# lyclyc52/Instance_NeRF

Measured on AMD Instinct MI355X. Metric: Msamples/sec (train+infer) 3D-FRONT 800x800 at 1/2/4/8 MI355X; PSNR parity, higher is better.
Workload: dtype f32; 1 GPU; render 800x800 synthetic 3D-FRONT-like room, hash-grid NeRF L=16 F=2 T=6119864 sigma+rgb (BASELINE configs[1]), one view per step per GPU; parallelism=views sharded over 1 GPU(s), no data-path collective

## Files before the change

instance_nerf_amd/build.py:

```python
import os
import shutil
import subprocess
import sys

HERE = os.path.dirname(os.path.abspath(__file__))
CSRC = os.path.join(HERE, "csrc")
LIB = os.path.join(CSRC, "libinr_hip.so")
SOURCES = ["raymarch.hip", "encoders.hip", "field_fused.hip", "roialign.hip", "mesh.hip", "components.hip", "match.hip",
           "overlap.hip"]
HEADERS = ["common.h", "grid_common.h", os.path.join("..", "..", "include", "inr.h")]
FLAGS = ["--offload-arch=gfx950", "-O3", "-std=c++17", "-fPIC", "-ffp-contract=off",
         "-munsafe-fp-atomics", "-Wall", "-Wno-unused-function"]


KERNEL_FILES = {
    "field": ["field_fused.hip", "common.h", "grid_common.h"],
    "scatter": ["encoders.hip", "common.h", "grid_common.h"],
}


def source_sha(kind=None):
    import hashlib
    h = hashlib.sha256()
    for f in sorted(KERNEL_FILES[kind] if kind else SOURCES + HEADERS):
        h.update(f.encode())
        h.update(open(os.path.join(CSRC, f), "rb").read())
    return h.hexdigest()


LIB_FP32 = os.path.join(CSRC, "libinr_hip_fp32.so")


def build_fp32(force=False, verbose=True):
    deps = [os.path.join(CSRC, f) for f in SOURCES + HEADERS] + [os.path.abspath(__file__)]
    if not force and os.path.exists(LIB_FP32) and all(os.path.getmtime(d) <= os.path.getmtime(LIB_FP32) for d in deps):
        return LIB_FP32
    hipcc = shutil.which("hipcc") or "/opt/rocm/bin/hipcc"
    objs = []
    for src in SOURCES:
        obj = os.path.join(CSRC, src.replace(".hip", ".fp32.o"))
        cmd = [hipcc, "-x", "hip", "-c", os.path.join(CSRC, src), "-o", obj, "-DINR_MLP_FP32=1"] + FLAGS
        if verbose:
            print(" ".join(cmd), flush=True)
        subprocess.check_call(cmd)
        objs.append(obj)
    subprocess.check_call([hipcc, "-shared", "-o", LIB_FP32] + objs + ["--offload-arch=gfx950"])
    return LIB_FP32


def _stale():
    if not os.path.exists(LIB):
        return True
    t = os.path.getmtime(LIB)
    deps = [os.path.join(CSRC, f) for f in SOURCES + HEADERS] + [os.path.abspath(__file__)]
    return any(os.path.getmtime(d) > t for d in deps)


def build(force=False, verbose=True):
    if not force and not _stale():
        return LIB
    hipcc = shutil.which("hipcc") or "/opt/rocm/bin/hipcc"
    if not os.path.exists(hipcc):
        raise RuntimeError("hipcc not found: cannot build libinr_hip.so")
    objs = []
    for src in SOURCES:
        obj = os.path.join(CSRC, src.replace(".hip", ".o"))
        cmd = [hipcc, "-x", "hip", "-c", os.path.join(CSRC, src), "-o", obj] + FLAGS
        if verbose:
            print(" ".join(cmd), flush=True)
        subprocess.check_call(cmd)
        objs.append(obj)
    cmd = [hipcc, "-shared", "-o", LIB] + objs + ["--offload-arch=gfx950"]
    if verbose:
        print(" ".join(cmd), flush=True)
    subprocess.check_call(cmd)
    return LIB


if __name__ == "__main__":
    build(force="--force" in sys.argv)
    build_fp32(force="--force" in sys.argv)
    print(LIB)
```

instance_nerf_amd/csrc/raymarch.hip:

```cpp
#include "common.h"

namespace inr {

static thread_local char g_err[512] = "";
int g_field_lds_min = 0;
int g_march_lds_pad = 0;
void set_error(const char* fmt, ...) {
  va_list ap;
  va_start(ap, fmt);
  vsnprintf(g_err, sizeof(g_err), fmt, ap);
  va_end(ap);
}

constexpr int kRayBlock = 256;
constexpr float kSqrt3x2 = 3.4641016151377544f;

__global__ void __launch_bounds__(kRayBlock) k_near_far(const float* __restrict__ rays_o,
                                                        const float* __restrict__ rays_d,
                                                        const float* __restrict__ aabb, int64_t N,
                                                        float min_near, float* __restrict__ nears,
                                                        float* __restrict__ fars,
                                                        const int64_t* __restrict__ labels, int64_t ignore) {
  const int64_t n = (int64_t)blockIdx.x * blockDim.x + threadIdx.x;
  if (n >= N) return;
  float near = -INFINITY, far = INFINITY;
  bool miss = labels != nullptr && labels[n] == ignore;
#pragma unroll
  for (int a = 0; a < 3; ++a) {
    const float o = rays_o[n * 3 + a];
    const float rd = 1.0f / rays_d[n * 3 + a];
    const float t0 = (aabb[a] - o) * rd;
    const float t1 = (aabb[a + 3] - o) * rd;
    const float lo = t0 > t1 ? t1 : t0;
    const float hi = t0 > t1 ? t0 : t1;
    if (a > 0) miss = miss || (near > hi) || (lo > far);
    near = lo > near ? lo : near;
    far = hi < far ? hi : far;
  }
  if (near < min_near) near = min_near;
  nears[n] = miss ? 3.402823466e+38f : near;
  fars[n] = miss ? 3.402823466e+38f : far;
}

__global__ void __launch_bounds__(kRayBlock) k_get_rays(const float* __restrict__ poses, int64_t B, float fx, float fy,
                                                        float cx, float cy, int W, const int64_t* __restrict__ inds,
                                                        int64_t n, float* __restrict__ rays_o,
                                                        float* __restrict__ rays_d) {
  const int64_t idx = (int64_t)blockIdx.x * blockDim.x + threadIdx.x;
  if (idx >= B * n) return;
  const int64_t b = idx / n, k = idx - b * n;
  const int64_t pix = inds ? inds[k] : k;
  const float i = (float)(pix % W) + 0.5f, j = (float)(pix / W) + 0.5f;
  const float xs = (i - cx) / fx, ys = (j - cy) / fy;
  const float nrm = sqrtf(xs * xs + ys * ys + 1.0f * 1.0f);
  const float dx = xs / nrm, dy = ys / nrm, dz = 1.0f / nrm;
  const float* P = poses + b * 16;
#pragma unroll
  for (int r = 0; r < 3; ++r) {
    rays_d[idx * 3 + r] = dx * P[r * 4 + 0] + dy * P[r * 4 + 1] + dz * P[r * 4 + 2];
    rays_o[idx * 3 + r] = P[r * 4 + 3];
  }
}

__device__ __forceinline__ uint64_t mix64(uint64_t z) {
  z = (z ^ (z >> 30)) * 0xBF58476D1CE4E5B9ull;
  z = (z ^ (z >> 27)) * 0x94D049BB133111EBull;
  return z ^ (z >> 31);
}
__global__ void __launch_bounds__(kRayBlock) k_sample_batch(const float* __restrict__ pose, float fx, float fy, float cx,
                                                            float cy, int H, int W, const float* __restrict__ image,
                                                            int C, const int32_t* __restrict__ mask, int num_instances,
                                                            uint64_t seed, uint64_t step, int64_t n,
                                                            int64_t* __restrict__ inds, float* __restrict__ rays_o,
                                                            float* __restrict__ rays_d, float* __restrict__ rgb,
                                                            int64_t* __restrict__ labels) {
  const int64_t k = (int64_t)blockIdx.x * blockDim.x + threadIdx.x;
  if (k >= n) return;
  const uint64_t h = mix64(seed + 0x9E3779B97F4A7C15ull * ((step << 32) + (uint64_t)k));
  const uint64_t pix = ((h >> 32) * (uint64_t)((int64_t)H * W)) >> 32;
  inds[k] = (int64_t)pix;
  const float i = (float)(pix % (uint64_t)W) + 0.5f, j = (float)(pix / (uint64_t)W) + 0.5f;
  const float xs = (i - cx) / fx, ys = (j - cy) / fy;
  const float nrm = sqrtf(xs * xs + ys * ys + 1.0f * 1.0f);
  const float dx = xs / nrm, dy = ys / nrm, dz = 1.0f / nrm;
#pragma unroll
  for (int r = 0; r < 3; ++r) {
    rays_d[k * 3 + r] = dx * pose[r * 4 + 0] + dy * pose[r * 4 + 1] + dz * pose[r * 4 + 2];
    rays_o[k * 3 + r] = pose[r * 4 + 3];
  }
  if (image) {
    for (int c = 0; c < C; ++c) rgb[k * C + c] = image[pix * C + c];
  }
  if (mask) {
    const int32_t l = mask[pix];
    labels[k] = l >= num_instances ? -1 : (int64_t)l;
  }
}

__global__ void k_morton3D(const int32_t* __restrict__ coords, int64_t N, int32_t* __restrict__ out) {
  const int64_t n = (int64_t)blockIdx.x * blockDim.x + threadIdx.x;
  if (n >= N) return;
  out[n] = (int32_t)morton3((uint32_t)coords[n * 3], (uint32_t)coords[n * 3 + 1], (uint32_t)coords[n * 3 + 2]);
}
__global__ void k_morton3D_invert(const int32_t* __restrict__ idx, int64_t N, int32_t* __restrict__ coords) {
  const int64_t n = (int64_t)blockIdx.x * blockDim.x + threadIdx.x;
  if (n >= N) return;
  const uint32_t m = (uint32_t)idx[n];
  coords[n * 3 + 0] = (int32_t)compact_bits10(m);
  coords[n * 3 + 1] = (int32_t)compact_bits10(m >> 1);
  coords[n * 3 + 2] = (int32_t)compact_bits10(m >> 2);
}
__global__ void k_packbits(const float* __restrict__ grid, int64_t n_bytes, float thresh,
                           uint8_t* __restrict__ bits) {
  const int64_t n = (int64_t)blockIdx.x * blockDim.x + threadIdx.x;
  if (n >= n_bytes) return;
  const float4 a = reinterpret_cast<const float4*>(grid)[n * 2];
  const float4 b = reinterpret_cast<const float4*>(grid)[n * 2 + 1];
  uint32_t v = (a.x > thresh) | ((a.y > thresh) << 1) | ((a.z > thresh) << 2) | ((a.w > thresh) << 3) |
               ((b.x > thresh) << 4) | ((b.y > thresh) << 5) | ((b.z > thresh) << 6) | ((b.w > thresh) << 7);
  bits[n] = (uint8_t)v;
}

__global__ void k_occ_positions(const int32_t* __restrict__ morton, const float* __restrict__ noise, int64_t n, float Hm1,
                                float ext, float half, float* __restrict__ xyz) {
  const int64_t i = (int64_t)blockIdx.x * blockDim.x + threadIdx.x;
  if (i >= n) return;
  const uint32_t m = morton ? (uint32_t)morton[i] : (uint32_t)i;
  const uint32_t c[3] = {compact_bits10(m), compact_bits10(m >> 1), compact_bits10(m >> 2)};
#pragma unroll
  for (int a = 0; a < 3; ++a) {
    float v = (2.0f * (float)c[a] / Hm1 - 1.0f) * ext;
    if (noise) v = v + (noise[i * 3 + a] * 2.0f - 1.0f) * half;
    xyz[i * 3 + a] = v;
  }
}
__global__ void __launch_bounds__(256) k_mark_untrained(const float* __restrict__ poses, int B, float kx, float ky, int H,
                                                        int C, float bound, float* __restrict__ grid) {
  const int64_t i = (int64_t)blockIdx.x * blockDim.x + threadIdx.x;
  const int64_t H3 = (int64_t)H * H * H;
  if (i >= (int64_t)C * H3) return;
  const int cas = (int)(i / H3);
  const uint32_t m = (uint32_t)(i - (int64_t)cas * H3);
  const float bnd = fminf(ldexpf(1.0f, cas), bound), half = bnd / (float)H, ext = bnd - half;
  const float wx = (2.0f * (float)compact_bits10(m) / (float)(H - 1) - 1.0f) * ext;
  const float wy = (2.0f * (float)compact_bits10(m >> 1) / (float)(H - 1) - 1.0f) * ext;
  const float wz = (2.0f * (float)compact_bits10(m >> 2) / (float)(H - 1) - 1.0f) * ext;
  bool seen = false;
  for (int b = 0; b < B && !seen; ++b) {
    const float* P = poses + (int64_t)b * 16;
    const float dx = wx - P[3], dy = wy - P[7], dz = wz - P[11];
    const float cx = dx * P[0] + dy * P[4] + dz * P[8];
    const float cy = dx * P[1] + dy * P[5] + dz * P[9];
    const float cz = dx * P[2] + dy * P[6] + dz * P[10];
    seen = cz > 0.0f && fabsf(cx) < kx * cz + half * 2.0f && fabsf(cy) < ky * cz + half * 2.0f;
  }
  if (!seen) grid[i] = -1.0f;
}

__global__ void k_occ_scatter(const float* __restrict__ sigma, const int32_t* __restrict__ morton, int64_t m,
                              float density_scale, float* __restrict__ tmp) {
  const int64_t i = (int64_t)blockIdx.x * blockDim.x + threadIdx.x;
  if (i < m) tmp[morton[i]] = sigma[i] * density_scale;
}
__global__ void __launch_bounds__(256) k_occ_update(float* __restrict__ grid, const float* __restrict__ tmp, int64_t n,
                                                    float decay, float scale, double* __restrict__ mean_sum) {
  __shared__ double red[4];
  double acc = 0.0;
  auto cell = [&](float g, float t, bool& changed) {
    t *= scale;
    if (g >= 0.0f && t >= 0.0f) { g = fmaxf(g * decay, t); changed = true; }
    acc += (double)fmaxf(g, 0.0f);
    return g;
  };
  const int64_t n4 = (((uintptr_t)grid | (uintptr_t)tmp) & 15) == 0 ? n / 4 : 0;
  for (int64_t i = (int64_t)blockIdx.x * blockDim.x + threadIdx.x; i < n4; i += (int64_t)gridDim.x * blockDim.x) {
    float4 g = reinterpret_cast<float4*>(grid)[i];
    const float4 t = reinterpret_cast<const float4*>(tmp)[i];
    bool changed = false;
    g.x = cell(g.x, t.x, changed); g.y = cell(g.y, t.y, changed); g.z = cell(g.z, t.z, changed); g.w = cell(g.w, t.w, changed);
    if (changed) reinterpret_cast<float4*>(grid)[i] = g;
  }
  for (int64_t i = n4 * 4 + (int64_t)blockIdx.x * blockDim.x + threadIdx.x; i < n; i += (int64_t)gridDim.x * blockDim.x) {
    bool changed = false;
    const float g = cell(grid[i], tmp[i], changed);
    if (changed) grid[i] = g;
  }
#pragma unroll
  for (int d = 32; d >= 1; d >>= 1) acc += __shfl_xor(acc, d, 64);
  if ((threadIdx.x & 63) == 0) red[threadIdx.x >> 6] = acc;
  __syncthreads();
  if (threadIdx.x == 0) atomicAdd(mean_sum, red[0] + red[1] + red[2] + red[3]);
}
__global__ void k_packbits_mean(const float* __restrict__ grid, int64_t n_bytes, const double* __restrict__ mean_sum,
                                double inv_cells, float density_thresh, uint8_t* __restrict__ bits,
                                float* __restrict__ mean_out, const int32_t* __restrict__ counters, int n_counters,
                                int counter_stride, double* __restrict__ stats_out) {
  const int64_t n = (int64_t)blockIdx.x * blockDim.x + threadIdx.x;
  const float mean = (float)(*mean_sum * inv_cells);
  if (n == 0 && mean_out) *mean_out = mean;
  if (n == 0 && stats_out) {
    int64_t total = 0;
    for (int k = 0; k < n_counters; ++k) total += counters[(int64_t)k * counter_stride];
    stats_out[0] = (double)mean;
    stats_out[1] = (double)total;
  }
  if (n >= n_bytes) return;
  const float thresh = fminf(mean, density_thresh);
  const float4 a = reinterpret_cast<const float4*>(grid)[n * 2];
  const float4 b = reinterpret_cast<const float4*>(grid)[n * 2 + 1];
  uint32_t v = (a.x > thresh) | ((a.y > thresh) << 1) | ((a.z > thresh) << 2) | ((a.w > thresh) << 3) |
               ((b.x > thresh) << 4) | ((b.y > thresh) << 5) | ((b.z > thresh) << 6) | ((b.w > thresh) << 7);
  bits[n] = (uint8_t)v;
}

struct MarchParams {
  const uint8_t* bits;
  float bound, dt_gamma, dt_min, dt_max, rH;
  int C, H, H3;
};

struct Ray {
  float ox, oy, oz, dx, dy, dz, rdx, rdy, rdz, sx, sy, sz;
};

__device__ __forceinline__ Ray load_ray(const float* __restrict__ o, const float* __restrict__ d, int64_t n) {
  Ray r;
  r.ox = o[n * 3]; r.oy = o[n * 3 + 1]; r.oz = o[n * 3 + 2];
  r.dx = d[n * 3]; r.dy = d[n * 3 + 1]; r.dz = d[n * 3 + 2];
  r.rdx = 1.0f / r.dx; r.rdy = 1.0f / r.dy; r.rdz = 1.0f / r.dz;
  r.sx = copysignf(1.0f, r.dx); r.sy = copysignf(1.0f, r.dy); r.sz = copysignf(1.0f, r.dz);
  return r;
}

__device__ __forceinline__ float step_dt(const MarchParams& P, float t) {
  return clampf(t * P.dt_gamma, P.dt_min, P.dt_max);
}
template <bool kConst>
struct StepRule {
  float c;
  __device__ __forceinline__ explicit StepRule(const MarchParams& P) : c(step_dt(P, 0.0f)) {}
  __device__ __forceinline__ float operator()(const MarchParams& P, float t) const {
    if constexpr (kConst) return c;
    else return step_dt(P, t);
  }
};

struct MortonCalc {
  __device__ __forceinline__ uint32_t operator()(uint32_t x, uint32_t y, uint32_t z) const { return morton3(x, y, z); }
};
struct MortonLut {
  const uint32_t* lut;
  __device__ __forceinline__ uint32_t operator()(uint32_t x, uint32_t y, uint32_t z) const {
    return lut[x] | (lut[y] << 1) | (lut[z] << 2);
  }
};

template <bool kSingle = false, bool kConstDt = false, class Emit, class Advance, class Morton = MortonCalc>
__device__ __forceinline__ int march_ray(const MarchParams& P, const Ray& r, float t, float far,
                                         int max_emit, Emit&& emit, Advance&& advance, Morton morton = Morton()) {
  int n = 0;
  float last_t = t;
  const StepRule<kConstDt> step(P);
  const float mb1 = fminf(ldexpf(1.0f, 0), P.bound), rmb1 = 1.0f / mb1;
  while (t < far && n < max_emit) {
    const float px = clampf(r.ox + t * r.dx, -P.bound, P.bound);
    const float py = clampf(r.oy + t * r.dy, -P.bound, P.bound);
    const float pz = clampf(r.oz + t * r.dz, -P.bound, P.bound);
    const float dt = step(P, t);
    int level = 0;
    float mb = mb1, rmb = rmb1;
    if constexpr (!kSingle) {
      int e0, e1;
      (void)frexpf(fmaxf(fabsf(px), fmaxf(fabsf(py), fabsf(pz))), &e0);
      (void)frexpf(dt * (float)P.H * 0.5f, &e1);
      level = max(clampi(e0, 0, P.C - 1), clampi(e1, 0, P.C - 1));
      mb = fminf(ldexpf(1.0f, level), P.bound);
      rmb = 1.0f / mb;
    }
    const int nx = clampi((int)(((px * rmb + 1.0f) * 0.5f) * (float)P.H), 0, P.H - 1);
    const int ny = clampi((int)(((py * rmb + 1.0f) * 0.5f) * (float)P.H), 0, P.H - 1);
    const int nz = clampi((int)(((pz * rmb + 1.0f) * 0.5f) * (float)P.H), 0, P.H - 1);
    const uint32_t idx = (uint32_t)level * (uint32_t)P.H3 + morton((uint32_t)nx, (uint32_t)ny, (uint32_t)nz);
    const bool occ = (P.bits[idx >> 3] >> (idx & 7)) & 1;
    if (occ) {
      const float tn = t + dt;
      emit(px, py, pz, dt, tn - last_t, t);
      t = tn;
      advance();
      last_t = tn;
      ++n;
    } else {
      const float ax = ((float)nx + 0.5f) + 0.5f * r.sx;
      const float ay = ((float)ny + 0.5f) + 0.5f * r.sy;
      const float az = ((float)nz + 0.5f) + 0.5f * r.sz;
      const float cx = (((ax * P.rH) * 2.0f - 1.0f) * mb - px) * r.rdx;
      const float cy = (((ay * P.rH) * 2.0f - 1.0f) * mb - py) * r.rdy;
      const float cz = (((az * P.rH) * 2.0f - 1.0f) * mb - pz) * r.rdz;
      const float tt = t + fmaxf(0.0f, fminf(cx, fminf(cy, cz)));
      do {
        t = t + step(P, t);
        advance();
      } while (t < tt);
    }
  }
  return n;
}
template <class Emit>
__device__ __forceinline__ int march_ray(const MarchParams& P, const Ray& r, float t, float far,
                                         int max_emit, Emit&& emit) {
  return P.dt_gamma == 0.0f ? march_ray<false, true>(P, r, t, far, max_emit, emit, [] {})
                            : march_ray<false, false>(P, r, t, far, max_emit, emit, [] {});
}
template <class Emit, class Advance, class Morton>
__device__ __forceinline__ int march_ray_any(const MarchParams& P, const Ray& r, float t, float far,
                                             int max_emit, Emit&& emit, Advance&& advance, Morton morton) {
  if (P.dt_gamma == 0.0f)
    return P.C == 1 ? march_ray<true, true>(P, r, t, far, max_emit, emit, advance, morton)
                    : march_ray<false, true>(P, r, t, far, max_emit, emit, advance, morton);
  return P.C == 1 ? march_ray<true, false>(P, r, t, far, max_emit, emit, advance, morton)
                  : march_ray<false, false>(P, r, t, far, max_emit, emit, advance, morton);
}

__device__ __forceinline__ float start_t(const MarchParams& P, float near, float noise) {
  return near + step_dt(P, near) * noise;
}

__global__ void __launch_bounds__(kRayBlock) k_march_count(MarchParams P, const float* __restrict__ rays_o,
                                                           const float* __restrict__ rays_d, int64_t N,
                                                           int max_steps, const float* __restrict__ nears,
                                                           const float* __restrict__ fars,
                                                           const float* __restrict__ noises,
                                                           int32_t* __restrict__ counts,
                                                           int32_t* __restrict__ block_sums,
                                                           uint32_t* __restrict__ mask, int cap_words) {
  __shared__ int32_t wsum[kRayBlock / 64];
  __shared__ uint32_t lut[1024];
  for (int i = threadIdx.x; i < P.H; i += kRayBlock) lut[i] = expand_bits10((uint32_t)i);
  __syncthreads();
  const MortonLut morton{lut};
  const int64_t n = (int64_t)blockIdx.x * blockDim.x + threadIdx.x;
  int cnt = 0;
  if (n < N) {
    const Ray r = load_ray(rays_o, rays_d, n);
    const float t0 = start_t(P, nears[n], noises ? noises[n] : 0.0f);
    if (cap_words > 0) {
      uint32_t word = 0;
      int widx = 0, cand = 0;
      bool ok = true;
      cnt = march_ray_any(P, r, t0, fars[n], max_steps,
                      [&](float, float, float, float, float, float) {
                        const int w = cand >> 5;
                        if (w < cap_words) {
                          while (widx < w) {
                            mask[(int64_t)widx * N + n] = word;
                            word = 0;
                            ++widx;
                          }
                          word |= 1u << (cand & 31);
                        } else {
                          ok = false;
                        }
                      },
                      [&] { ++cand; }, morton);
      if (widx < cap_words) mask[(int64_t)widx * N + n] = word;
      mask[(int64_t)cap_words * N + n] = ok ? 1u : 0u;
    } else {
      cnt = march_ray_any(P, r, t0, fars[n], max_steps, [](float, float, float, float, float, float) {}, [] {}, morton);
    }
    counts[n] = cnt;
  }
  const int incl = wave_inclusive_scan(cnt);
  if ((threadIdx.x & 63) == 63) wsum[threadIdx.x >> 6] = incl;
  __syncthreads();
  if (threadIdx.x == 0) {
    int s = 0;
#pragma unroll
    for (int w = 0; w < kRayBlock / 64; ++w) s += wsum[w];
    block_sums[blockIdx.x] = s;
  }
}

__global__ void __launch_bounds__(1024) k_scan_block_sums(int32_t* __restrict__ block_sums, int n_blocks,
                                                          int64_t N, int32_t* __restrict__ counter) {
  __shared__ int32_t wsum[16];
  __shared__ int32_t carry_s;
  if (threadIdx.x == 0) carry_s = 0;
  __syncthreads();
  for (int base = 0; base < n_blocks; base += 1024) {
    const int i = base + threadIdx.x;
    const int v = i < n_blocks ? block_sums[i] : 0;
    const int incl = wave_inclusive_scan(v);
    if ((threadIdx.x & 63) == 63) wsum[threadIdx.x >> 6] = incl;
    __syncthreads();
    int wave_off = 0;
    for (int w = 0; w < (int)(threadIdx.x >> 6); ++w) wave_off += wsum[w];
    const int carry = carry_s;
    if (i < n_blocks) block_sums[i] = carry + wave_off + incl - v;
    __syncthreads();
    if (threadIdx.x == 1023) carry_s = carry + wave_off + incl;
    __syncthreads();
  }
  if (threadIdx.x == 0) {
    counter[0] = carry_s;
    counter[1] = (int32_t)N;
  }
}

__global__ void __launch_bounds__(kRayBlock) k_finalize_offsets(const int32_t* __restrict__ counts,
                                                                const int32_t* __restrict__ block_prefix,
                                                                int64_t N, int32_t* __restrict__ rays) {
  __shared__ int32_t wsum[kRayBlock / 64];
  const int64_t n = (int64_t)blockIdx.x * blockDim.x + threadIdx.x;
  const int cnt = n < N ? counts[n] : 0;
  const int incl = wave_inclusive_scan(cnt);
  if ((threadIdx.x & 63) == 63) wsum[threadIdx.x >> 6] = incl;
  __syncthreads();
  int off = block_prefix[blockIdx.x] + incl - cnt;
  for (int w = 0; w < (int)(threadIdx.x >> 6); ++w) off += wsum[w];
  if (n < N) {
    rays[n * 3 + 0] = (int32_t)n;
    rays[n * 3 + 1] = off;
    rays[n * 3 + 2] = cnt;
  }
}

template <bool kConstDt, class Emit>
__device__ __forceinline__ void replay_ray_t(const MarchParams& P, const Ray& r, const uint32_t* __restrict__ mask, int64_t N,
                                             int64_t n, float t, int cnt, Emit&& emit) {
  const StepRule<kConstDt> step(P);
  float last_t = t;
  int emitted = 0;
  for (int w = 0; emitted < cnt; ++w) {
    const uint32_t bits = mask[(int64_t)w * N + n];
    for (int b0 = 0; b0 < 32; b0 += 8) {
      const uint32_t sub = (bits >> b0) & 0xFFu;
      if (__ballot(sub != 0u) == 0ull) {
#pragma unroll
        for (int j = 0; j < 8; ++j) t = t + step(P, t);
        continue;
      }
#pragma unroll
      for (int j = 0; j < 8; ++j) {
        const float dt = step(P, t);
        const float tn = t + dt;
        if (sub & (1u << j)) {
          const float px = clampf(r.ox + t * r.dx, -P.bound, P.bound);
          const float py = clampf(r.oy + t * r.dy, -P.bound, P.bound);
          const float pz = clampf(r.oz + t * r.dz, -P.bound, P.bound);
          emit(px, py, pz, dt, tn - last_t, t);
          last_t = tn;
          ++emitted;
        }
        t = tn;
      }
    }
  }
}
template <class Emit>
__device__ __forceinline__ void replay_ray(const MarchParams& P, const Ray& r, const uint32_t* __restrict__ mask, int64_t N,
                                           int64_t n, float t, int cnt, Emit&& emit) {
  if (P.dt_gamma == 0.0f) replay_ray_t<true>(P, r, mask, N, n, t, cnt, emit);
  else replay_ray_t<false>(P, r, mask, N, n, t, cnt, emit);
}

__global__ void __launch_bounds__(kRayBlock) k_march_write(MarchParams P, const float* __restrict__ rays_o,
                                                           const float* __restrict__ rays_d, int64_t N,
                                                           int64_t M, const float* __restrict__ nears,
                                                           const float* __restrict__ fars,
                                                           const float* __restrict__ noises,
                                                           const int32_t* __restrict__ rays,
                                                           float* __restrict__ xyzs, float* __restrict__ dirs,
                                                           float* __restrict__ deltas,
                                                           const uint32_t* __restrict__ mask, int cap_words) {
  const int64_t n = (int64_t)blockIdx.x * blockDim.x + threadIdx.x;
  if (n >= N) return;
  const int off = rays[n * 3 + 1];
  const int cnt = rays[n * 3 + 2];
  if (cnt == 0 || (int64_t)off + cnt > M) return;
  const Ray r = load_ray(rays_o, rays_d, n);
  int64_t i = off;
  auto emit = [&](float px, float py, float pz, float dt, float delta, float) {
    xyzs[i * 3 + 0] = px; xyzs[i * 3 + 1] = py; xyzs[i * 3 + 2] = pz;
    dirs[i * 3 + 0] = r.dx; dirs[i * 3 + 1] = r.dy; dirs[i * 3 + 2] = r.dz;
    deltas[i * 2 + 0] = dt; deltas[i * 2 + 1] = delta;
    ++i;
  };
  const float t0 = start_t(P, nears[n], noises ? noises[n] : 0.0f);
  if (cap_words > 0 && mask[(int64_t)cap_words * N + n]) {
    replay_ray(P, r, mask, N, n, t0, cnt, emit);
  } else {
    march_ray(P, r, t0, fars[n], cnt, emit);
  }
}

template <bool kSingle = false, class Emit>
__device__ __forceinline__ int march_ray_coop(const MarchParams& P, const Ray& r, float t, float far, int max_emit,
                                              Emit&& emit) {
  const float mb1 = fminf(ldexpf(1.0f, 0), P.bound), rmb1 = 1.0f / mb1;
  const int lane = threadIdx.x & 63;
  const uint64_t lt_mask = (1ull << lane) - 1ull;
  int n = 0;
  float last_t = t;
  while (t < far && n < max_emit) {
    float c = t;
    if (P.dt_gamma == 0.0f) {
      const float dt0 = step_dt(P, t);
      asm volatile(
          ".rept 63\n"
          "s_nop 1\n"
          "v_add_f32_dpp %0, %0, %1 wave_shr:1 row_mask:0xf bank_mask:0xf\n"
          ".endr\n"
          : "+v"(c)
          : "v"(dt0));
    } else {
      for (int j = 0; j < 63; ++j) c = j < lane ? c + step_dt(P, c) : c;
    }
    const bool in = c < far;
    const float px = clampf(r.ox + c * r.dx, -P.bound, P.bound);
    const float py = clampf(r.oy + c * r.dy, -P.bound, P.bound);
    const float pz = clampf(r.oz + c * r.dz, -P.bound, P.bound);
    const float dt = step_dt(P, c);
    const float tn = c + dt;
    int level = 0;
    float mb = mb1, rmb = rmb1;
    if constexpr (!kSingle) {
      int e0, e1;
      (void)frexpf(fmaxf(fabsf(px), fmaxf(fabsf(py), fabsf(pz))), &e0);
      (void)frexpf(dt * (float)P.H * 0.5f, &e1);
      level = max(clampi(e0, 0, P.C - 1), clampi(e1, 0, P.C - 1));
      mb = fminf(ldexpf(1.0f, level), P.bound);
      rmb = 1.0f / mb;
    }
    const int nx = clampi((int)(((px * rmb + 1.0f) * 0.5f) * (float)P.H), 0, P.H - 1);
    const int ny = clampi((int)(((py * rmb + 1.0f) * 0.5f) * (float)P.H), 0, P.H - 1);
    const int nz = clampi((int)(((pz * rmb + 1.0f) * 0.5f) * (float)P.H), 0, P.H - 1);
    const uint32_t idx = (uint32_t)level * (uint32_t)P.H3 + morton3((uint32_t)nx, (uint32_t)ny, (uint32_t)nz);
    const bool occ = (P.bits[idx >> 3] >> (idx & 7)) & 1;
    const float ax = ((float)nx + 0.5f) + 0.5f * r.sx;
    const float ay = ((float)ny + 0.5f) + 0.5f * r.sy;
    const float az = ((float)nz + 0.5f) + 0.5f * r.sz;
    const float cx = (((ax * P.rH) * 2.0f - 1.0f) * mb - px) * r.rdx;
    const float cy = (((ay * P.rH) * 2.0f - 1.0f) * mb - py) * r.rdy;
    const float cz = (((az * P.rH) * 2.0f - 1.0f) * mb - pz) * r.rdz;
    const float tt = c + fmaxf(0.0f, fminf(cx, fminf(cy, cz)));
    int lo = lane + 1, hi = 64;
    bool settled_all = false;
    if (P.dt_gamma == 0.0f) {
      const int i0 = lane + (int)fminf((tt - c) * (1.0f / dt), 64.0f);
      const float ca = __shfl(c, clampi(i0 - 1, 0, 63), 64);
      const float cb = __shfl(c, min(i0, 63), 64);
      const float cc = __shfl(c, min(i0 + 1, 63), 64);
      const bool lt_a = i0 - 1 <= lane || ca < tt;
      const bool ge_b = i0 >= 64 || !(cb < tt);
      const bool ge_c = i0 + 1 >= 64 || !(cc < tt);
      const bool take_b = i0 > lane && ge_b;
      const bool settled = take_b ? lt_a : ge_c;
      lo = take_b ? min(i0, 64) : i0 + 1;
      settled_all = __ballot(in && !occ && !settled) == 0;
    }
    if (!settled_all) {
      lo = lane + 1;
#pragma unroll
      for (int it = 0; it < 7; ++it) {
        const int mid = (lo + hi) >> 1;
        const float cm = __shfl(c, min(mid, 63), 64);
        const bool below = mid < 64 && cm < tt;
        if (lo < hi) {
          if (below) lo = mid + 1; else hi = mid;
        }
      }
    }
    const int next = lo;
    const uint64_t in_mask = __ballot(in);
    const uint64_t miss_mask = __ballot(in && !occ);
    const int n_in = __popcll(in_mask);
    uint64_t visited = 0;
    int v = 0, last_miss = -1;
    while (v < n_in) {
      const uint64_t rest = miss_mask >> v;
      const int m = rest ? v + __builtin_ctzll(rest) : 64;
      const int stop = min(m, n_in);
      if (stop > v) visited |= (stop - v >= 64 ? ~0ull : ((1ull << (stop - v)) - 1ull)) << v;
      if (m >= n_in) { v = stop; last_miss = -1; break; }
      visited |= 1ull << m;
      last_miss = m;
      v = __builtin_amdgcn_readlane(next, m);
    }
    uint64_t emit_mask = visited & in_mask & ~miss_mask;
    int k_new = __popcll(emit_mask);
    bool full = false;
    if (n + k_new >= max_emit) {
      full = true;
      const int keep = max_emit - n;
      uint64_t m2 = emit_mask;
      for (int i = 0; i < keep; ++i) m2 &= m2 - 1;
      emit_mask &= ~m2;
      k_new = keep;
    }
    const uint64_t before = emit_mask & lt_mask;
    const int prev = before ? 63 - __builtin_clzll(before) : 0;
    const float prev_tn = __shfl(tn, prev, 64);
    if ((emit_mask >> lane) & 1ull) {
      const float last = before ? prev_tn : last_t;
      emit(n + __popcll(before), px, py, pz, dt, tn - last, c);
    }
    if (emit_mask) last_t = __builtin_bit_cast(float, __builtin_amdgcn_readlane(__builtin_bit_cast(int, tn),
                                                                                63 - __builtin_clzll(emit_mask)));
    n += k_new;
    if (full) break;
    if (v < 64) {
      t = far;
    } else {
      const float c63 = __builtin_bit_cast(float, __builtin_amdgcn_readlane(__builtin_bit_cast(int, tn), 63));
      t = c63;
      if (last_miss >= 0) {
        const float tt_m = __builtin_bit_cast(float, __builtin_amdgcn_readlane(__builtin_bit_cast(int, tt), last_miss));
        while (t < tt_m) t = t + step_dt(P, t);
      }
    }
  }
  return n;
}

constexpr int kCoopRaysPerBlock = 4;

__global__ void __launch_bounds__(kCoopRaysPerBlock * 64) k_march_count_coop(MarchParams P, const float* __restrict__ rays_o,
                                                                             const float* __restrict__ rays_d, int64_t N,
                                                                             int max_steps, const float* __restrict__ nears,
                                                                             const float* __restrict__ fars,
                                                                             const float* __restrict__ noises,
                                                                             int32_t* __restrict__ counts,
                                                                             float* __restrict__ stage, int stage_pitch) {
  const int64_t n = (int64_t)blockIdx.x * kCoopRaysPerBlock + (threadIdx.x >> 6);
  if (n >= N) return;
  const Ray r = load_ray(rays_o, rays_d, n);
  const float t0 = start_t(P, nears[n], noises ? noises[n] : 0.0f);
  int cnt;
  if (stage) {
    float* row = stage + (size_t)n * stage_pitch * 5;
    auto park = [&](int k, float px, float py, float pz, float dt, float delta, float) {
      float* q = row + (size_t)k * 5;
      q[0] = px; q[1] = py; q[2] = pz; q[3] = dt; q[4] = delta;
    };
    cnt = P.C == 1 ? march_ray_coop<true>(P, r, t0, fars[n], max_steps, park)
                   : march_ray_coop<false>(P, r, t0, fars[n], max_steps, park);
  } else {
    auto none = [](int, float, float, float, float, float, float) {};
    cnt = P.C == 1 ? march_ray_coop<true>(P, r, t0, fars[n], max_steps, none)
                   : march_ray_coop<false>(P, r, t0, fars[n], max_steps, none);
  }
  if ((threadIdx.x & 63) == 0) counts[n] = cnt;
}

__global__ void __launch_bounds__(kCoopRaysPerBlock * 64) k_march_write_staged(const float* __restrict__ rays_d, int64_t N,
                                                                               int64_t M, const int32_t* __restrict__ rays,
                                                                               const float* __restrict__ stage, int stage_pitch,
                                                                               float* __restrict__ xyzs, float* __restrict__ dirs,
                                                                               float* __restrict__ deltas) {
  const int64_t n = (int64_t)blockIdx.x * kCoopRaysPerBlock + (threadIdx.x >> 6);
  if (n >= N) return;
  const int off = rays[n * 3 + 1];
  const int cnt = rays[n * 3 + 2];
  const int lane = threadIdx.x & 63;
  auto zero_rows = [&](int64_t lo, int64_t hi) {
    for (int64_t i = lo + lane; i < hi; i += 64) {
      xyzs[i * 3 + 0] = 0.f; xyzs[i * 3 + 1] = 0.f; xyzs[i * 3 + 2] = 0.f;
      dirs[i * 3 + 0] = 0.f; dirs[i * 3 + 1] = 0.f; dirs[i * 3 + 2] = 0.f;
      deltas[i * 2 + 0] = 0.f; deltas[i * 2 + 1] = 0.f;
    }
  };
  const int64_t total = (int64_t)rays[(N - 1) * 3 + 1] + rays[(N - 1) * 3 + 2];
  if (total < M) {
    const int64_t per = (M - total + N - 1) / N;
    zero_rows(total + n * per, min(M, total + (n + 1) * per));
  }
  if ((int64_t)off + cnt > M) {
    if (cnt > 0 && off < M) zero_rows(off, M);
    return;
  }
  if (cnt == 0) return;
  const float dx = rays_d[n * 3], dy = rays_d[n * 3 + 1], dz = rays_d[n * 3 + 2];
  const float* row = stage + (size_t)n * stage_pitch * 5;
  for (int k = lane; k < cnt; k += 64) {
    const float* q = row + (size_t)k * 5;
    const int64_t i = (int64_t)off + k;
    xyzs[i * 3 + 0] = q[0]; xyzs[i * 3 + 1] = q[1]; xyzs[i * 3 + 2] = q[2];
    dirs[i * 3 + 0] = dx; dirs[i * 3 + 1] = dy; dirs[i * 3 + 2] = dz;
    deltas[i * 2 + 0] = q[3]; deltas[i * 2 + 1] = q[4];
  }
}

constexpr int kOccBuckets = 4096;
constexpr int kOccBlockCells = 1024;
constexpr int kOccMaxBlocks = 16384;
__global__ void __launch_bounds__(kOccBlockCells) k_occ_count(const float* __restrict__ grid, int64_t n_cells,
                                                              uint64_t* __restrict__ masks, int32_t* __restrict__ block_counts,
                                                              int32_t* __restrict__ hist) {
  __shared__ int32_t wcount[kOccBlockCells / 64];
  const int64_t i = (int64_t)blockIdx.x * kOccBlockCells + threadIdx.x;
  const uint64_t m = __ballot(i < n_cells && grid[i] > 0.0f);
  if ((threadIdx.x & 63) == 0) {
    masks[i >> 6] = m;
    wcount[threadIdx.x >> 6] = __popcll(m);
  }
  for (int64_t k = i; k < 2 * kOccBuckets; k += (int64_t)gridDim.x * kOccBlockCells) hist[k] = 0;
  __syncthreads();
  if (threadIdx.x == 0) {
    int c = 0;
    for (int w = 0; w < kOccBlockCells / 64; ++w) c += wcount[w];
    block_counts[blockIdx.x] = c;
  }
}
__global__ void __launch_bounds__(1024) k_occ_hist(const float* __restrict__ u, int64_t n, int32_t* __restrict__ hist) {
  __shared__ int32_t h[2 * kOccBuckets];
  for (int k = threadIdx.x; k < 2 * kOccBuckets; k += 1024) h[k] = 0;
  __syncthreads();
  for (int64_t j = (int64_t)blockIdx.x * 1024 + threadIdx.x; j < 2 * n; j += (int64_t)gridDim.x * 1024) {
    const int b = min((int)(u[j] * (float)kOccBuckets), kOccBuckets - 1);
    atomicAdd(&h[(j >= n ? kOccBuckets : 0) + b], 1);
  }
  __syncthreads();
  for (int k = threadIdx.x; k < 2 * kOccBuckets; k += 1024)
    if (h[k]) atomicAdd(&hist[k], h[k]);
}
__device__ void lds_exclusive_scan_1024(int32_t* a, int n, int32_t* wsum) {
  const int per = (n + 1023) / 1024;
  const int lo = min(n, (int)threadIdx.x * per), hi = min(n, lo + per);
  int s = 0;
  for (int i = lo; i < hi; ++i) s += a[i];
  const int incl = wave_inclusive_scan(s);
  if ((threadIdx.x & 63) == 63) wsum[threadIdx.x >> 6] = incl;
  __syncthreads();
// ... 1297 lines not shown
```

Baseline: 6442 Msamples/s.

## Replace per-step float marching in empty space with closed-form binade jumps

Adds a ConstStepper that, for constant step size, computes how many float additions of the step fit within the current exponent binade and jumps there in closed form using fma, so the result stays bit-exact with repeated t+=c. Empty-space skipping in march_ray and the mask replay in replay_ray_t use it, with replay jumping straight to each set bit via ctz instead of stepping through every candidate. The goal is to cut the long serial add loops over skipped samples. In exchange the per-ray code is more complex and branchy, and bit-exactness depends on subtle rounding handling.

```diff
diff --git a/instance_nerf_amd/build.py b/instance_nerf_amd/build.py
--- a/instance_nerf_amd/build.py
+++ b/instance_nerf_amd/build.py
@@ -8,7 +8,7 @@
 LIB = os.path.join(CSRC, "libinr_hip.so")
 SOURCES = ["raymarch.hip", "encoders.hip", "field_fused.hip", "roialign.hip", "mesh.hip", "components.hip", "match.hip",
            "overlap.hip"]
-HEADERS = ["common.h", "grid_common.h", os.path.join("..", "..", "include", "inr.h")]
+HEADERS = ["common.h", "grid_common.h", "const_step.h", os.path.join("..", "..", "include", "inr.h")]
 FLAGS = ["--offload-arch=gfx950", "-O3", "-std=c++17", "-fPIC", "-ffp-contract=off",
          "-munsafe-fp-atomics", "-Wall", "-Wno-unused-function"]
 
diff --git a/instance_nerf_amd/csrc/const_step.h b/instance_nerf_amd/csrc/const_step.h
--- /dev/null
+++ b/instance_nerf_amd/csrc/const_step.h
@@ -0,0 +1,126 @@
+#pragma once
+#include <math.h>
+#include <stdint.h>
+
+#if defined(__HIPCC__) || defined(__CUDACC__)
+#define INR_STEP_HD __host__ __device__ __forceinline__
+#else
+#define INR_STEP_HD inline
+#endif
+
+namespace inr {
+
+struct ConstStepper {
+  float c;
+  uint32_t eb = 0;
+  float q = 0.0f, rq = 0.0f, top = 0.0f;
+  bool plain = true;
+
+  static constexpr float kMaxJump = 32768.0f;
+
+  INR_STEP_HD explicit ConstStepper(float step) : c(step) {}
+
+  static INR_STEP_HD uint32_t bits_of(float x) {
+    uint32_t b;
+    __builtin_memcpy(&b, &x, sizeof b);
+    return b;
+  }
+  static INR_STEP_HD float float_of(uint32_t b) {
+    float x;
+    __builtin_memcpy(&x, &b, sizeof x);
+    return x;
+  }
+  static INR_STEP_HD bool covered(uint32_t e) { return e - 32u <= 190u; }
+
+  INR_STEP_HD void set_binade(uint32_t e) {
+    eb = e;
+    const float u = float_of((e - 23u) << 23), ru = float_of((277u - e) << 23);
+    top = float_of((e + 1u) << 23);
+    const float s = c * ru;
+    const float m = rintf(s);
+    q = m * u;
+    plain = !(fabsf(s - m) != 0.5f) || !(q > 0.0f);
+    rq = 1.0f / q;
+  }
+  INR_STEP_HD bool tie_or_stuck(uint32_t e) {
+    set_binade(e);
+    return plain;
+  }
+
+  INR_STEP_HD bool closed_form_at(float t, float* room) {
+    const uint32_t e = bits_of(t) >> 23;
+    if (!covered(e)) return false;
+    if (e != eb) set_binade(e);
+    *room = top - t;
+    return !plain && q <= *room;
+  }
+
+  INR_STEP_HD float advance_to(float t, float tt, int* steps) {
+    for (;;) {
+      float room;
+      if (!closed_form_at(t, &room)) {
+        t = t + c;
+        ++*steps;
+      } else {
+        const float lim = top < tt ? top : tt;
+        float kf = ceilf((lim - t) * rq);
+        kf = kf > 1.0f ? kf : 1.0f;
+        if (!(kf < kMaxJump)) {
+          t = t + c;
+          ++*steps;
+        } else {
+          float tk = fmaf(kf, q, t);
+          while (tk < lim) {
+            kf += 1.0f;
+            tk = fmaf(kf, q, t);
+          }
+          while (kf > 1.0f) {
+            const float tp = fmaf(kf - 1.0f, q, t);
+            if (!(tp >= lim)) break;
+            kf -= 1.0f;
+            tk = tp;
+          }
+          if (fmaf(kf, q, -room) > 0.0f) {
+            kf -= 1.0f;
+            t = fmaf(kf, q, t);
+            t = t + c;
+            *steps += (int)kf + 1;
+          } else {
+            t = tk;
+            *steps += (int)kf;
+          }
+        }
+      }
+      if (!(t < tt)) return t;
+    }
+  }
+
+  INR_STEP_HD float nth(float t, int k) {
+    while (k > 0) {
+      float room;
+      if (!closed_form_at(t, &room)) {
+        t = t + c;
+        --k;
+        continue;
+      }
+      const int kk = k < (int)kMaxJump ? k : (int)kMaxJump;
+      const float kf = (float)kk;
+      if (fmaf(kf, q, -room) <= 0.0f) {
+        t = fmaf(kf, q, t);
+        k -= kk;
+        continue;
+      }
+      float jf = floorf(room * rq);
+      jf = jf < kf - 1.0f ? jf : kf - 1.0f;
+      jf = jf > 1.0f ? jf : 1.0f;
+      while (fmaf(jf, q, -room) > 0.0f) jf -= 1.0f;
+      while (fmaf(jf + 1.0f, q, -room) <= 0.0f) jf += 1.0f;
+      t = fmaf(jf, q, t);
+      t = t + c;
+      k -= (int)jf + 1;
+    }
+    return t;
+  }
+};
+
+}
diff --git a/instance_nerf_amd/csrc/raymarch.hip b/instance_nerf_amd/csrc/raymarch.hip
--- a/instance_nerf_amd/csrc/raymarch.hip
+++ b/instance_nerf_amd/csrc/raymarch.hip
@@ -1,4 +1,7 @@
+#include <type_traits>
+
 #include "common.h"
+#include "const_step.h"
 
 namespace inr {
 
@@ -255,12 +258,19 @@
   }
 };
 
+template <class Advance>
+__device__ __forceinline__ void advance_by(Advance&& advance, int k) {
+  if constexpr (std::is_invocable_v<Advance&, int>) advance(k);
+  else for (int i = 0; i < k; ++i) advance();
+}
+
 template <bool kSingle = false, bool kConstDt = false, class Emit, class Advance, class Morton = MortonCalc>
 __device__ __forceinline__ int march_ray(const MarchParams& P, const Ray& r, float t, float far,
                                          int max_emit, Emit&& emit, Advance&& advance, Morton morton = Morton()) {
   int n = 0;
   float last_t = t;
   const StepRule<kConstDt> step(P);
+  [[maybe_unused]] ConstStepper jump(step.c);
   const float mb1 = fminf(ldexpf(1.0f, 0), P.bound), rmb1 = 1.0f / mb1;
   while (t < far && n < max_emit) {
     const float px = clampf(r.ox + t * r.dx, -P.bound, P.bound);
@@ -286,7 +296,7 @@
       const float tn = t + dt;
       emit(px, py, pz, dt, tn - last_t, t);
       t = tn;
-      advance();
+      advance_by(advance, 1);
       last_t = tn;
       ++n;
     } else {
@@ -297,10 +307,16 @@
       const float cy = (((ay * P.rH) * 2.0f - 1.0f) * mb - py) * r.rdy;
       const float cz = (((az * P.rH) * 2.0f - 1.0f) * mb - pz) * r.rdz;
       const float tt = t + fmaxf(0.0f, fminf(cx, fminf(cy, cz)));
-      do {
-        t = t + step(P, t);
-        advance();
-      } while (t < tt);
+      if constexpr (kConstDt) {
+        int k = 0;
+        t = jump.advance_to(t, tt, &k);
+        advance_by(advance, k);
+      } else {
+        do {
+          t = t + step(P, t);
+          advance_by(advance, 1);
+        } while (t < tt);
+      }
     }
   }
   return n;
@@ -361,7 +377,7 @@
                           ok = false;
                         }
                       },
-                      [&] { ++cand; }, morton);
+                      [&](int k) { cand += k; }, morton);
       if (widx < cap_words) mask[(int64_t)widx * N + n] = word;
       mask[(int64_t)cap_words * N + n] = ok ? 1u : 0u;
     } else {
@@ -428,6 +444,30 @@
 __device__ __forceinline__ void replay_ray_t(const MarchParams& P, const Ray& r, const uint32_t* __restrict__ mask, int64_t N,
                                              int64_t n, float t, int cnt, Emit&& emit) {
   const StepRule<kConstDt> step(P);
+  if constexpr (kConstDt) {
+    ConstStepper jump(step.c);
+    float last_t = t;
+    int emitted = 0, at = 0;
+    for (int w = 0; emitted < cnt; ++w) {
+      uint32_t bits = mask[(int64_t)w * N + n];
+      while (bits) {
+        const int idx = (w << 5) + __builtin_ctz(bits);
+        bits &= bits - 1u;
+        t = jump.nth(t, idx - at);
+        const float dt = step(P, t);
+        const float tn = t + dt;
+        const float px = clampf(r.ox + t * r.dx, -P.bound, P.bound);
+        const float py = clampf(r.oy + t * r.dy, -P.bound, P.bound);
+        const float pz = clampf(r.oz + t * r.dz, -P.bound, P.bound);
+        emit(px, py, pz, dt, tn - last_t, t);
+        last_t = tn;
+        t = tn;
+        at = idx + 1;
+        ++emitted;
+      }
+    }
+    return;
+  }
   float last_t = t;
   int emitted = 0;
   for (int w = 0; emitted < cnt; ++w) {
```

New measurement: 6473 Msamples/s (median of 6 runs). About the same (+0.5%).
